# amikey/kaldi-ctc

Measured on AMD Instinct MI355X. Metric: CTC-train frames/sec, 5×BLSTM-512 mb=16, at 1/2/4/8 MI355X; loss match, higher is better.
Workload: dtype f32

## Files before the change

### include/ctc.h

```cpp
#ifndef KALDI_CTC_AMD_CTC_H_
#define KALDI_CTC_AMD_CTC_H_

#include <stddef.h>

#ifdef __cplusplus
extern "C" {
#endif

struct ihipStream_t;
typedef struct ihipStream_t *ctcStream_t;

typedef enum {
  CTC_STATUS_SUCCESS = 0,
  CTC_STATUS_MEMOPS_FAILED = 1,
  CTC_STATUS_INVALID_VALUE = 2,
  CTC_STATUS_EXECUTION_FAILED = 3,
  CTC_STATUS_UNKNOWN_ERROR = 4
} ctcStatus_t;

typedef enum { CTC_CPU = 0, CTC_GPU = 1 } ctcComputeLocation;

struct ctcOptions {
  ctcComputeLocation loc;
  union {
    unsigned int num_threads;
    ctcStream_t stream;
  };
  int blank_label;
};

int get_warpctc_version(void);
const char *ctcGetStatusString(ctcStatus_t status);

ctcStatus_t compute_ctc_loss(const float *const activations, float *gradients,
                             const int *const flat_labels, const int *const label_lengths,
                             const int *const input_lengths, int alphabet_size,
                             int minibatch, float *costs, void *workspace,
                             struct ctcOptions options);

ctcStatus_t get_workspace_size(const int *const label_lengths,
                               const int *const input_lengths, int alphabet_size,
                               int minibatch, struct ctcOptions info,
                               size_t *size_bytes);

ctcStatus_t mictc_compute_ctc_loss_async(const float *activations, float *gradients,
                                         const int *flat_labels, const int *label_lengths,
                                         const int *input_lengths, int alphabet_size,
                                         int minibatch, double *costs_dev, void *workspace,
                                         ctcStream_t stream, int blank_label);

int mictc_set_frame_group(int m);

int mictc_set_win(int on);

#ifdef __cplusplus
}
#endif
#endif
```

### kaldi-ctc_amd/__init__.py

```python
import ctypes
import os

import numpy as np

HERE = os.path.dirname(os.path.abspath(__file__))
LIB_PATH = os.path.join(HERE, "libkaldictc_amd.so")

CTC_CPU, CTC_GPU = 0, 1
CTC_STATUS = {0: "CTC_STATUS_SUCCESS", 1: "CTC_STATUS_MEMOPS_FAILED", 2: "CTC_STATUS_INVALID_VALUE",
              3: "CTC_STATUS_EXECUTION_FAILED", 4: "CTC_STATUS_UNKNOWN_ERROR"}

_lib = None


class CtcOptions(ctypes.Structure):
    _fields_ = [("loc", ctypes.c_int), ("stream", ctypes.c_void_p), ("blank_label", ctypes.c_int)]


class CtcError(RuntimeError):
    def __init__(self, status, where):
        msg = lib().ctcGetStatusString(status).decode()
        super().__init__(f"ctcStatus_t {status} : \"{msg}\" returned from '{where}'")
        self.status = status

# ... 86 lines not shown
    ll = np.ascontiguousarray(label_lengths, dtype=np.int32)
    il = np.ascontiguousarray(input_lengths, dtype=np.int32)
    opts = CtcOptions(CTC_GPU, None, 0)
    out = ctypes.c_size_t()
    st = lib().get_workspace_size(ll.ctypes.data, il.ctypes.data, int(alphabet_size), len(ll),
                                  opts, ctypes.byref(out))
    if st != 0:
        raise CtcError(st, "get_workspace_size")
    return out.value


def compute_ctc_loss(acts, flat_labels, label_lengths, input_lengths, want_grad=True, blank=0,
                     stream=None, workspace=None):
    import torch
    assert acts.is_cuda and acts.dtype == torch.float32 and acts.is_contiguous()
    T, N, A = acts.shape
    fl = np.ascontiguousarray(flat_labels, dtype=np.int32)
    if fl.size == 0:
        fl = np.zeros(1, np.int32)
    ll = np.ascontiguousarray(label_lengths, dtype=np.int32)
    il = np.ascontiguousarray(input_lengths, dtype=np.int32)
    if workspace is None:
        workspace = torch.empty(ctc_workspace_size(ll, il, A), dtype=torch.uint8, device=acts.device)
    grads = torch.empty_like(acts) if want_grad else None
    costs = np.zeros(N, np.float32)
    opts = CtcOptions(CTC_GPU, _stream_handle(stream), blank)
    st = lib().compute_ctc_loss(acts.data_ptr(), _ptr(grads), fl.ctypes.data, ll.ctypes.data,
                                il.ctypes.data, A, N, costs.ctypes.data, workspace.data_ptr(), opts)
    if st != 0:
        raise CtcError(st, "compute_ctc_loss")
    return costs, grads


class RnnError(RuntimeError):
    pass


def _krnn_check(st, where):
    if st != 0:
        raise RnnError(f"{where}: {lib().krnnGetStatusString(st).decode()} ({st})")


class Rnn:
    RELU, TANH, LSTM, GRU = 0, 1, 2, 3

    def __init__(self, mode, input_dim, hidden_dim, num_layers=1, bidirectional=True):
        self.mode, self.D, self.H, self.L = mode, input_dim, hidden_dim, num_layers
        self.dirs = 2 if bidirectional else 1
        h = ctypes.c_void_p()
        _krnn_check(lib().krnnCreate(ctypes.byref(h), mode, input_dim, hidden_dim, num_layers,
                                     1 if bidirectional else 0), "krnnCreate")
        self.h = h

    def set_precision(self, prec):
        _krnn_check(lib().krnnSetPrecision(self.h, 1 if prec in (1, "bf16") else 0), "krnnSetPrecision")

    def __del__(self):
        try:
            if self.h:
                lib().krnnDestroy(self.h)
        except Exception:
            pass

    @property
    def num_params(self):
        return lib().krnnGetParamsSize(self.h) // 4
# ... 904 lines not shown
```

### kaldi-ctc_amd/_bindings.py

```python
import ctypes

vp, ci, cl, cf, cd, sz = (ctypes.c_void_p, ctypes.c_int, ctypes.c_long, ctypes.c_float,
                          ctypes.c_double, ctypes.c_size_t)
ip = ctypes.POINTER(ctypes.c_int)

SIGS = {
    "krnnCreate": (ci, [ctypes.POINTER(vp), ci, ci, ci, ci, ci]),
    "krnnDestroy": (ci, [vp]),
    "krnnGetStatusString": (ctypes.c_char_p, [ci]),
    "krnnGetParamsSize": (sz, [vp]),
    "krnnGetLinLayerOffset": (cl, [vp, ci, ci, ci, ip]),
    "krnnGetWorkspaceSize": (sz, [vp, ci, ci]),
    "krnnGetTrainingReserveSize": (sz, [vp, ci, ci]),
    "krnnForwardTraining": (ci, [vp, vp, ci, ci, vp, vp, vp, vp, sz, vp, sz]),
    "krnnForwardInference": (ci, [vp, vp, ci, ci, vp, vp, vp, vp, sz]),
    "krnnGetInferenceSeqWorkspaceSize": (sz, [vp, ci, ci]),
    "krnnForwardInferenceSeq": (ci, [vp, vp, ci, ci, vp, vp, vp, vp, vp, sz]),
    "krnnBackwardData": (ci, [vp, vp, ci, ci, vp, vp, vp, vp, vp, sz, vp, sz]),
    "krnnBackwardWeights": (ci, [vp, vp, ci, ci, vp, vp, vp, sz, vp, vp, sz]),
    "krnnGetDeviceStatus": (ci, [vp, vp]),
    "kcm_add_mat_mat": (ci, [vp, ci, ci, ci, ci, ci, cf, vp, cl, vp, cl, cf, vp, cl]),
    "kcm_add_mat_mat_x3_workspace": (sz, [ci, ci, ci]),
    "kcm_add_mat_mat_x3": (ci, [vp, ci, ci, ci, ci, ci, cf, vp, cl, vp, cl, cf, vp, cl, vp]),
    "kcm_bench_gemm_packed": (cf, [vp, ci, ci, ci, ci, ci, ci]),
    "kcm_test_gemm_packed": (ci, [vp, ci, ci, ci, ci, ci, ci, ci, ci, vp, vp, vp, vp]),
    "kcm_test_row_stream": (ci, [vp, ci, ci, ci, ci, ci, vp, vp, vp, vp]),
    "kctc_test_component_side_streams": (ci, [vp, ci]),
    "kctc_test_rec6_select": (ci, [ci, ci, ci, ci, ci, ci, ip, ctypes.POINTER(vp)]),
    "kctc_test_rec_plan": (ci, [ci, ci, ci, ci, ci, ci, ctypes.POINTER(cl)]),
    "kcm_find_row_max_id": (ci, [vp, vp, cl, ci, vp]),
    "kcm_clip_gradient_rows": (ci, [vp, vp, cl, ci, cf, vp]),
    "kcm_add_vec_clipped": (ci, [vp, vp, vp, cl, cf, cf]),
    "kcm_add_row_sum_mat": (ci, [vp, vp, cl, ci, cf, cf, vp, vp]),
    "kctc_last_error": (ctypes.c_char_p, []),
    "kctc_nnet_create": (ci, [ctypes.POINTER(vp), ctypes.c_char_p, ctypes.c_ulonglong, ci]),
    "kctc_nnet_destroy": (ci, [vp]),
    "kctc_nnet_num_components": (ci, [vp]),
    "kctc_nnet_context": (ci, [vp, ip, ip]),
    "kctc_nnet_component_info": (ci, [vp, ci, ctypes.c_char_p, sz]),
    "kctc_nnet_num_params": (cl, [vp, ci]),
    "kctc_nnet_get_params": (ci, [vp, ci, vp, cl]),
    "kctc_nnet_set_params": (ci, [vp, ci, vp, cl]),
    "kctc_nnet_get_grad": (ci, [vp, ci, vp, cl]),
    "kctc_nnet_set_learning_rate": (ci, [vp, cf]),
    "kctc_nnet_clip_stats": (ci, [vp, ci, ctypes.POINTER(cd), ctypes.POINTER(cd)]),
    "kctc_nnet_srand": (ci, [vp, ctypes.c_uint]),
    "kctc_nnet_rand_calls": (ci, [vp, ctypes.POINTER(cl)]),
    "kctc_nnet_last_best_path": (ci, [vp, vp, cl]),
    "kctc_nnet_last_output": (ci, [vp, vp, cl]),
    "kctc_nnet_last_costs": (ci, [vp, vp, ci]),
    "kctc_nnet_train_step": (ci, [vp, vp, ci, ci, vp, vp, vp, ctypes.POINTER(cd), ctypes.POINTER(cd),
                                  ctypes.POINTER(cd)]),
    "kctc_nnet_compute_objf": (ci, [vp, vp, ci, ci, vp, vp, vp, ctypes.POINTER(cd), ctypes.POINTER(cd),
                                    ctypes.POINTER(cd)]),
    "kctc_nnet_train_step_async": (ci, [vp, vp, ci, ci, vp, vp, vp, ip, ctypes.POINTER(cd), ctypes.POINTER(cd),
                                        ctypes.POINTER(cd)]),
    "kctc_nnet_train_flush": (ci, [vp, ip, ctypes.POINTER(cd), ctypes.POINTER(cd), ctypes.POINTER(cd)]),
    "kctc_nnet_stream": (vp, [vp]),
    "kctc_nnet_set_profiling": (ci, [vp, ci]),
    "kctc_nnet_profile": (ci, [vp, ctypes.c_char_p, ctypes.POINTER(cd), ctypes.POINTER(ci)]),
    "kctc_nnet_write": (ci, [vp, ctypes.c_char_p]),
    "kctc_nnet_read": (ci, [ctypes.POINTER(vp), ctypes.c_char_p, ci]),
# ... 98 lines not shown
```

### kaldi-ctc_amd/csrc/common.h

```cpp
#pragma once
#include <hip/hip_runtime.h>

#include <cmath>
#include <cstdint>
#include <cstdio>
#include <stdexcept>
#include <string>

namespace kctc {

constexpr int kWave = 64;

struct HipError : std::runtime_error {
  explicit HipError(const std::string &s) : std::runtime_error(s) {}
};

#define KCTC_HIP_CHECK(expr)                                                          \
  do {                                                                                \
    hipError_t e_ = (expr);                                                           \
    if (e_ != hipSuccess)                                                             \
      throw ::kctc::HipError(std::string(#expr) + ": " + hipGetErrorString(e_) + " @" \
                             + __FILE__ + ":" + std::to_string(__LINE__));            \
  } while (0)

// ... 10 lines not shown
  for (int o = 32; o >= 1; o >>= 1) v = fmaxf(v, __shfl_xor(v, o, kWave));
  return v;
}
#define KCTC_DPP(v, ctrl, rm) \
  __int_as_float(__builtin_amdgcn_update_dpp(__float_as_int(v), __float_as_int(v), ctrl, rm, 0xF, false))
__device__ __forceinline__ float group_max8(float v) {
  v = fmaxf(v, KCTC_DPP(v, 0xB1, 0xF));
  v = fmaxf(v, KCTC_DPP(v, 0x4E, 0xF));
  v = fmaxf(v, KCTC_DPP(v, 0x141, 0xF));
  return v;
}
__device__ __forceinline__ float group_max16(float v) {
  v = group_max8(v);
  return fmaxf(v, KCTC_DPP(v, 0x140, 0xF));
}
__device__ __forceinline__ float wave_max_l63(float v) {
  v = group_max16(v);
  v = fmaxf(v, KCTC_DPP(v, 0x142, 0xA));
  v = fmaxf(v, KCTC_DPP(v, 0x143, 0xC));
  return v;
}

__device__ __forceinline__ float wave_sum(float v) {
#pragma unroll
  for (int o = 32; o >= 1; o >>= 1) v += __shfl_xor(v, o, kWave);
  return v;
}
__device__ __forceinline__ double wave_sum_d(double v) {
#pragma unroll
  for (int o = 32; o >= 1; o >>= 1) v += __shfl_xor(v, o, kWave);
  return v;
}

}
```

### kaldi-ctc_amd/csrc/ctc.hip

```cpp
#include <algorithm>
#include <cstring>
#include <type_traits>
#include <atomic>
#include <vector>

#include "common.h"
#include "ctc.h"
#include "prof.h"

namespace kctc {
namespace ctcimpl {

constexpr int kMaxLabel = 639;
constexpr int kThreads = 256;
constexpr int kABThreads = 512;
constexpr int kABWaves = kABThreads / 64;
constexpr int kSPT = (2 * kMaxLabel + 1 + kABThreads - 1) / kABThreads;
constexpr int kFR = 8;

struct UttDesc {
  int T, L, S, feasible, lab_off, pad;
  long long ab_off;
  long long off_off;
};

struct Layout {
  size_t desc, labels, links, owner, costs, logz, lp, spill, offs, total;
  int T_max;
  long long spill_floats, off_doubles;
};

static bool make_layout(const int *label_lengths, const int *input_lengths, int A, int N,
                        Layout *lay, std::vector<UttDesc> *descs, bool *bad) {
  *bad = false;
  if (A <= 0 || N <= 0 || !label_lengths || !input_lengths) { *bad = true; return false; }
  int T_max = 0;
  long long nlab = 0, spill = 0, offs = 0;
  if (descs) descs->resize(N);
  for (int n = 0; n < N; n++) {
    int T = input_lengths[n], L = label_lengths[n];
    if (T < 0 || L < 0 || L > kMaxLabel) { *bad = true; return false; }
    T_max = T > T_max ? T : T_max;
    int S = 2 * L + 1;
    if (descs) {
      UttDesc &d = (*descs)[n];
      d.T = T; d.L = L; d.S = S; d.feasible = 0; d.lab_off = (int)nlab; d.pad = 0;
      d.ab_off = spill; d.off_off = offs;
    }
    nlab += L;
    spill += 2LL * T * S;
    offs += 2LL * T;
  }
  Layout &l = *lay;
  size_t p = 0;
  l.desc = p;   p = align_up(p + sizeof(UttDesc) * N, 256);
  l.labels = p; p = align_up(p + sizeof(int) * (nlab > 0 ? nlab : 1), 256);
  l.links = p;  p = align_up(p + sizeof(int) * (nlab > 0 ? nlab : 1), 256);
  l.owner = p;  p = align_up(p + sizeof(int) * (size_t)N * A, 256);
  l.costs = p;  p = align_up(p + sizeof(double) * N, 256);
  l.logz = p;   p = align_up(p + sizeof(float) * (size_t)T_max * N + 4, 256);
  l.lp = p;     p = align_up(p + sizeof(float) * (size_t)T_max * N * A + 4, 256);
  l.spill = p;  p = align_up(p + sizeof(float) * (size_t)spill, 256);
  l.offs = p;   p = align_up(p + sizeof(double) * (size_t)offs, 256);
  l.total = p;
  l.T_max = T_max;
  l.spill_floats = spill;
  l.off_doubles = offs;
  return true;
}

__global__ __launch_bounds__(256) void ctc_logz(const float *__restrict__ acts, int A, long rows,
                                                float *__restrict__ logz, float *__restrict__ lp) {
  const long row = (long)blockIdx.x * 4 + (threadIdx.x >> 6);
  const int lane = threadIdx.x & 63;
  if (row >= rows) return;
  const float *r = acts + row * A;
  float m = -INFINITY;
  for (int a = lane; a < A; a += kWave) m = fmaxf(m, r[a]);
  m = wave_max(m);
  float s = 0.f;
  for (int a = lane; a < A; a += kWave) s += expf(r[a] - m);
  s = wave_sum(s);
  const float z = m + logf(s);
  if (lane == 0) logz[row] = z;
  for (int a = lane; a < A; a += kWave) lp[row * A + a] = r[a] - z;
}

__device__ __forceinline__ float fast_log1p(float x) {
  const float u = 1.f + x;
  return __builtin_fmaf(__builtin_amdgcn_logf(u), 0.693147180559945309f, x - (u - 1.f));
}
__device__ __forceinline__ float lse3(float a, float b, float c) {
  const float m = fmaxf(a, fmaxf(b, c));
  const float lo = fminf(a, fminf(b, c));
  const float md = fmaxf(fminf(a, b), fminf(fmaxf(a, b), c));
  const float r = m + fast_log1p(__expf(md - m) + __expf(lo - m));
  return m == -INFINITY ? -INFINITY : r;
}

struct AbLds {
  int F, SP, CP;
  int pair;
  __device__ __host__ size_t floats() const { return 2 * (size_t)F * SP + 2 * (size_t)CP + 2 * kABWaves + 4; }
};

__device__ __forceinline__ void lds_barrier() {
  asm volatile("s_waitcnt lgkmcnt(0)" ::: "memory");
  __builtin_amdgcn_s_barrier();
  asm volatile("" ::: "memory");
}

template <bool SPILL, int SPT, bool is_beta>
__device__ __forceinline__ void ab_body(
    const float *__restrict__ lp, int N, int A, int blank, UttDesc *__restrict__ descs,
    const int *__restrict__ labels, float *__restrict__ spill, double *__restrict__ offs,
    double *__restrict__ costs, AbLds lay) {
  const int n = is_beta ? blockIdx.x - N : blockIdx.x;
  const int tid = threadIdx.x, lane = tid & 63, wid = tid >> 6;
// ... 366 lines not shown
    lds_barrier();
  }
  if (!is_beta && tid == 0) {
    const float *pv = colb + (cur ^ 1) * CP;
    float a = pv[S - 1], b = S > 1 ? pv[S - 2] : -INFINITY;
    float m = fmaxf(a, b);
    double lpv = off + (double)m + log((double)expf(a - m) + (double)expf(b - m));
    costs[n] = -lpv;
  }
}

template <bool SPILL>
__global__ __launch_bounds__(64 * kWinWaves) void ctc_alpha_beta_win(
    const float *__restrict__ lp, int N, int A, int blank, UttDesc *__restrict__ descs,
    const int *__restrict__ labels, float *__restrict__ spill, double *__restrict__ offs,
    double *__restrict__ costs, AbLds lay) {
  if (blockIdx.x >= (unsigned)N) win_body<SPILL, true>(lp, N, A, blank, descs, labels, spill, offs, costs, lay);
  else win_body<SPILL, false>(lp, N, A, blank, descs, labels, spill, offs, costs, lay);
}

template <bool SPILL, int SPT>
__global__ __launch_bounds__(kABThreads) void ctc_alpha_beta(
    const float *__restrict__ lp, int N, int A, int blank, UttDesc *__restrict__ descs,
    const int *__restrict__ labels, float *__restrict__ spill, double *__restrict__ offs,
    double *__restrict__ costs, AbLds lay) {
  if (blockIdx.x >= (unsigned)N) ab_body<SPILL, SPT, true>(lp, N, A, blank, descs, labels, spill, offs, costs, lay);
  else ab_body<SPILL, SPT, false>(lp, N, A, blank, descs, labels, spill, offs, costs, lay);
}

__global__ __launch_bounds__(kThreads) void ctc_grad(
    const float *__restrict__ acts, const float *__restrict__ logz, float *__restrict__ grads,
    int N, int A, int T_max, int blank, const UttDesc *__restrict__ descs,
    const int *__restrict__ links, const int *__restrict__ owners, const float *__restrict__ spill,
    const double *__restrict__ offs, const double *__restrict__ costs) {
  extern __shared__ __attribute__((aligned(16))) char smem[];
  const int n = blockIdx.y, t0 = blockIdx.x * kFR, tid = threadIdx.x;
  const UttDesc d = descs[n];
  const int T = d.feasible ? d.T : 0, L = d.L, S = d.S;
  const int nf = min(kFR, T_max - t0);
  if (t0 >= T) {
    for (int it = tid; it < nf * A; it += kThreads) {
      int f = it / A, a = it - f * A;
      grads[((long)(t0 + f) * N + n) * A + a] = 0.f;
    }
    return;
  }
  float *occ = reinterpret_cast<float *>(smem);
  int *nxt = reinterpret_cast<int *>(occ + kFR * S);
  int *owner = nxt + (L > 0 ? L : 1);
  float *gblank = reinterpret_cast<float *>(owner + A);
  float *gtot = gblank + kFR;
  for (int a = tid; a < A; a += kThreads) owner[a] = owners[(long)n * A + a];
  for (int j = tid; j < L; j += kThreads) nxt[j] = links[d.lab_off + j];
  const double logp = -costs[n];
  const float *al = spill + d.ab_off;
  const float *be = al + (long long)T * S;
  const double *oa = offs + d.off_off, *ob = oa + T;
  const int nreal = min(nf, T - t0);
  for (int f = 0; f < nreal; f++) {
    const int t = t0 + f;
    const float Kt = (float)(oa[t] + ob[t] - logp);
    for (int s = tid; s < S; s += kThreads) {
      float v = al[(long)t * S + s] + be[(long)t * S + s];
      occ[f * S + s] = (v == -INFINITY) ? 0.f : expf(v + Kt);
    }
  }
  __syncthreads();
  {
    const int lane = tid & 63, wid = tid >> 6;
    for (int f = wid; f < nreal; f += kThreads / kWave) {
      float acc = 0.f, tot = 0.f;
      for (int s = 2 * lane; s < S; s += 2 * kWave) {
        acc += occ[f * S + s];
        tot += occ[f * S + s] + (s + 1 < S ? occ[f * S + s + 1] : 0.f);
      }
      acc = wave_sum(acc);
      tot = wave_sum(tot);
      if (lane == 0) { gblank[f] = acc / tot; gtot[f] = 1.f / tot; }
    }
  }
  __syncthreads();
  for (int it = tid; it < nf * A; it += kThreads) {
    const int f = it / A, a = it - f * A, t = t0 + f;
    const long idx = ((long)t * N + n) * A + a;
    float g = 0.f;
    if (t < T) {
      float gam = 0.f;
      if (a == blank) {
        gam = gblank[f];
      } else {
        for (int j = owner[a]; j >= 0; j = nxt[j]) gam += occ[f * S + 2 * j + 1];
        gam *= gtot[f];
      }
      g = expf(acts[idx] - logz[(long)t * N + n]) - gam;
    }
    grads[idx] = g;
  }
}

struct Staging {
  char *buf = nullptr;
  size_t cap = 0;
  hipEvent_t ev = nullptr;
  bool pending = false;
};
static thread_local Staging g_stage;

static char *staging_acquire(size_t bytes) {
  Staging &s = g_stage;
  if (s.pending) {
    if (hipEventSynchronize(s.ev) != hipSuccess) return nullptr;
    s.pending = false;
  }
  if (!s.ev && hipEventCreateWithFlags(&s.ev, hipEventDisableTiming) != hipSuccess) return nullptr;
  if (bytes > s.cap) {
    if (s.buf) (void)hipHostFree(s.buf);
    size_t cap = align_up(bytes * 2, 4096);
    if (hipHostMalloc((void **)&s.buf, cap, hipHostMallocDefault) != hipSuccess) {
      s.buf = nullptr; s.cap = 0;
      return nullptr;
    }
    s.cap = cap;
  }
  return s.buf;
}
static void staging_release(hipStream_t stream) {
  if (hipEventRecord(g_stage.ev, stream) == hipSuccess) g_stage.pending = true;
}

static std::atomic<int> g_frame_group{0};
static int frame_group() {
  int m = g_frame_group.load(std::memory_order_relaxed);
  if (m <= 0) {
    m = 8;
    int expect = 0;
    g_frame_group.compare_exchange_strong(expect, m);
    m = g_frame_group.load(std::memory_order_relaxed);
  }
  return m;
}

static std::atomic<int> g_win{1};
static bool win_enabled() { return g_win.load(std::memory_order_relaxed) != 0; }

static ctcStatus_t launch(const float *acts, float *grads, const int *flat_labels,
                          const int *label_lengths, const int *input_lengths, int A, int N,
                          double *costs_dev, void *workspace, hipStream_t stream, int blank) {
  Layout lay;
  std::vector<UttDesc> descs;
  bool bad = false;
  if (!make_layout(label_lengths, input_lengths, A, N, &lay, &descs, &bad) || bad)
    return CTC_STATUS_INVALID_VALUE;
  if (blank < 0 || blank >= A || !acts || !workspace) return CTC_STATUS_INVALID_VALUE;
  long long nlab = 0;
  for (int n = 0; n < N; n++) nlab += label_lengths[n];
  for (long long i = 0; i < nlab; i++)
    if (flat_labels[i] < 0 || flat_labels[i] >= A || flat_labels[i] == blank)
      return CTC_STATUS_INVALID_VALUE;
  char *ws = static_cast<char *>(workspace);
  char *stage = staging_acquire(lay.costs);
  if (!stage) return CTC_STATUS_MEMOPS_FAILED;
  memcpy(stage + lay.desc, descs.data(), sizeof(UttDesc) * N);
  if (nlab) memcpy(stage + lay.labels, flat_labels, sizeof(int) * nlab);
  {
    int *links = reinterpret_cast<int *>(stage + lay.links), *owner = reinterpret_cast<int *>(stage + lay.owner);
    std::fill(owner, owner + (size_t)N * A, -1);
    long long off = 0;
    for (int n = 0; n < N; n++) {
      const int L = label_lengths[n];
      int *own = owner + (size_t)n * A;
      for (int j = L - 1; j >= 0; j--) {
        const int k = flat_labels[off + j];
        links[off + j] = own[k];
        own[k] = j;
      }
      off += L;
    }
  }
  if (hipMemcpyAsync(ws, stage, lay.costs, hipMemcpyHostToDevice, stream) != hipSuccess)
    return CTC_STATUS_MEMOPS_FAILED;
  staging_release(stream);
  UttDesc *d_desc = reinterpret_cast<UttDesc *>(ws + lay.desc);
  const int *d_lab = reinterpret_cast<const int *>(ws + lay.labels);
  float *d_logz = reinterpret_cast<float *>(ws + lay.logz);
  float *d_spill = reinterpret_cast<float *>(ws + lay.spill);
  double *d_offs = reinterpret_cast<double *>(ws + lay.offs);
  const long rows = (long)lay.T_max * N;
  float *d_lp = reinterpret_cast<float *>(ws + lay.lp);
  if (rows > 0) {
    ProfSpan ps(stream, "ctc_logz");
    hipLaunchKernelGGL(ctc_logz, dim3(ceil_div(rows, 4)), dim3(256), 0, stream, acts, A, rows,
                       d_logz, d_lp);
  }
  const int want = grads != nullptr;
  {
    int Smax = 1;
    for (int n = 0; n < N; n++) Smax = 2 * label_lengths[n] + 1 > Smax ? 2 * label_lengths[n] + 1 : Smax;
    AbLds al;
    al.pair = frame_group();
    al.SP = (Smax + 63) / 64 * 64;
    const int own = 64 - 2 * (std::max(1, std::min(al.pair, 8)) - 1);
    const int nwv = std::max(1, (Smax + own - 1) / own);
    if (nwv <= kWinWaves && win_enabled()) {
      al.CP = std::max((Smax + 4 + 3) / 4 * 4, own * nwv);
      al.F = (int)std::min<size_t>(32, std::max<size_t>(4, (size_t)96 * 1024 / (2 * sizeof(float) * al.SP)));
      const size_t shm = sizeof(float) * (2 * (size_t)al.F * al.SP + 2 * (size_t)al.CP + 2 * kWinWaves + 4);
      if (shm > 160 * 1024) return CTC_STATUS_INVALID_VALUE;
      ProfSpan ps(stream, "ctc_alpha_beta");
      auto kern = want ? ctc_alpha_beta_win<true> : ctc_alpha_beta_win<false>;
      (void)hipFuncSetAttribute(reinterpret_cast<const void *>(kern), hipFuncAttributeMaxDynamicSharedMemorySize,
                                (int)shm);
      hipLaunchKernelGGL(kern, dim3(want ? 2 * N : N), dim3(64 * nwv), shm, stream, d_lp, N, A, blank, d_desc, d_lab,
                         d_spill, d_offs, costs_dev, al);
    } else {
      al.CP = std::max((Smax + 4 + 3) / 4 * 4, (Smax <= kABThreads ? 1 : kSPT) * kABThreads);
      al.F = (int)std::min<size_t>(32, std::max<size_t>(4, (size_t)96 * 1024 / (2 * sizeof(float) * al.SP)));
      const size_t shm = sizeof(float) * al.floats();
      if (shm > 160 * 1024) return CTC_STATUS_INVALID_VALUE;
      ProfSpan ps(stream, "ctc_alpha_beta");
      auto go = [&](auto kern, int grid) {
        (void)hipFuncSetAttribute(reinterpret_cast<const void *>(kern), hipFuncAttributeMaxDynamicSharedMemorySize,
                                  (int)shm);
        hipLaunchKernelGGL(kern, dim3(grid), dim3(kABThreads), shm, stream, d_lp, N, A, blank, d_desc, d_lab,
                           d_spill, d_offs, costs_dev, al);
      };
      if (Smax <= kABThreads) {
        if (want) go(ctc_alpha_beta<true, 1>, 2 * N);
        else go(ctc_alpha_beta<false, 1>, N);
      } else {
        if (want) go(ctc_alpha_beta<true, kSPT>, 2 * N);
        else go(ctc_alpha_beta<false, kSPT>, N);
      }
    }
  }
  if (want && lay.T_max > 0) {
    int Lmax = 0;
    for (int n = 0; n < N; n++) Lmax = label_lengths[n] > Lmax ? label_lengths[n] : Lmax;
    const int Smax = 2 * Lmax + 1;
    size_t shm = sizeof(float) * kFR * Smax + sizeof(int) * (Lmax > 0 ? Lmax : 1) +
                 sizeof(int) * A + 2 * sizeof(float) * kFR;
    if (shm > 160 * 1024) return CTC_STATUS_INVALID_VALUE;
    ProfSpan ps(stream, "ctc_grad");
    hipLaunchKernelGGL(ctc_grad, dim3(ceil_div(lay.T_max, kFR), N), dim3(kThreads), shm, stream,
                       acts, d_logz, grads, N, A, lay.T_max, blank, d_desc,
                       reinterpret_cast<const int *>(ws + lay.links), reinterpret_cast<const int *>(ws + lay.owner),
                       d_spill, d_offs, costs_dev);
  }
  if (hipGetLastError() != hipSuccess) return CTC_STATUS_EXECUTION_FAILED;
  return CTC_STATUS_SUCCESS;
}

}
}

using namespace kctc::ctcimpl;

extern "C" {

int get_warpctc_version(void) { return 2; }

int mictc_set_frame_group(int m) {
  const int prev = frame_group();
  if (m > 0) g_frame_group.store(std::max(1, std::min(m, 8)));
  return prev;
}

int mictc_set_win(int on) {
  const int prev = g_win.load();
  if (on >= 0) g_win.store(on ? 1 : 0);
  return prev;
}

const char *ctcGetStatusString(ctcStatus_t status) {
  switch (status) {
    case CTC_STATUS_SUCCESS: return "no error";
    case CTC_STATUS_MEMOPS_FAILED: return "cuda memcpy or memset failed";
    case CTC_STATUS_INVALID_VALUE: return "invalid value";
    case CTC_STATUS_EXECUTION_FAILED: return "execution failed";
    case CTC_STATUS_UNKNOWN_ERROR:
    default: return "unknown error";
  }
}

ctcStatus_t get_workspace_size(const int *const label_lengths, const int *const input_lengths,
                               int alphabet_size, int minibatch, struct ctcOptions info,
                               size_t *size_bytes) {
  if (!size_bytes || info.loc != CTC_GPU) return CTC_STATUS_INVALID_VALUE;
  Layout lay;
  bool bad = false;
  if (!make_layout(label_lengths, input_lengths, alphabet_size, minibatch, &lay, nullptr, &bad) ||
      bad)
    return CTC_STATUS_INVALID_VALUE;
  *size_bytes = lay.total;
  return CTC_STATUS_SUCCESS;
}

ctcStatus_t mictc_compute_ctc_loss_async(const float *activations, float *gradients,
                                         const int *flat_labels, const int *label_lengths,
                                         const int *input_lengths, int alphabet_size,
                                         int minibatch, double *costs_dev, void *workspace,
                                         ctcStream_t stream, int blank_label) {
  if (!costs_dev) return CTC_STATUS_INVALID_VALUE;
  try {
    return launch(activations, gradients, flat_labels, label_lengths, input_lengths,
                  alphabet_size, minibatch, costs_dev, workspace,
                  reinterpret_cast<hipStream_t>(stream), blank_label);
  } catch (...) {
    return CTC_STATUS_UNKNOWN_ERROR;
  }
}

ctcStatus_t compute_ctc_loss(const float *const activations, float *gradients,
                             const int *const flat_labels, const int *const label_lengths,
                             const int *const input_lengths, int alphabet_size, int minibatch,
                             float *costs, void *workspace, struct ctcOptions options) {
  if (options.loc != CTC_GPU || !costs) return CTC_STATUS_INVALID_VALUE;
  Layout lay;
  bool bad = false;
  if (!make_layout(label_lengths, input_lengths, alphabet_size, minibatch, &lay, nullptr, &bad) ||
      bad)
    return CTC_STATUS_INVALID_VALUE;
  hipStream_t stream = reinterpret_cast<hipStream_t>(options.stream);
  double *d_costs = reinterpret_cast<double *>(static_cast<char *>(workspace) + lay.costs);
  ctcStatus_t st = mictc_compute_ctc_loss_async(activations, gradients, flat_labels,
                                                label_lengths, input_lengths, alphabet_size,
                                                minibatch, d_costs, workspace, options.stream,
                                                options.blank_label);
  if (st != CTC_STATUS_SUCCESS) return st;
  std::vector<double> hc(minibatch);
  if (hipMemcpyAsync(hc.data(), d_costs, sizeof(double) * minibatch, hipMemcpyDeviceToHost,
                     stream) != hipSuccess)
    return CTC_STATUS_MEMOPS_FAILED;
  if (hipStreamSynchronize(stream) != hipSuccess) return CTC_STATUS_EXECUTION_FAILED;
  for (int n = 0; n < minibatch; n++) costs[n] = (float)hc[n];
  return CTC_STATUS_SUCCESS;
}

}
```

### kaldi-ctc_amd/csrc/elementwise.hip

```cpp
#include "common.h"
#include "elementwise.h"

namespace kctc {
namespace {

typedef float floatx4 __attribute__((ext_vector_type(4)));

__global__ __launch_bounds__(256) void k_clip_sgd(float *__restrict__ w, const float *__restrict__ dw,
                                                  long n, float lr, float clip, const unsigned *skip) {
  if (skip && *skip) return;
  const long n4 = n / 4;
  const long stride = (long)gridDim.x * 256;
  const bool vec = ((uintptr_t)w % 16 == 0) && ((uintptr_t)dw % 16 == 0);
  long i = (long)blockIdx.x * 256 + threadIdx.x;
  if (vec) {
    for (; i < n4; i += stride) {
      floatx4 g = reinterpret_cast<const floatx4 *>(dw)[i];
      floatx4 v = reinterpret_cast<floatx4 *>(w)[i];
#pragma unroll
      for (int j = 0; j < 4; j++) {
        float x = g[j];
        if (clip > 0.f) x = fminf(fmaxf(x, -clip), clip);
        v[j] += lr * x;
      }
// ... 24 lines not shown
        ss += v[0] * v[0] + v[1] * v[1] + v[2] * v[2] + v[3] * v[3];
      }
    } else {
      for (int j = lane; j < dim; j += 64) ss += r[j] * r[j];
    }
    ss = wave_sum(ss);
    const float sc = ss * inv_thr2;
    if (!(sc < 1.f)) {
      clipped = 1;
      const float f = rsqrtf(sc);
      if (vec) {
        for (int j = lane; j < dim / 4; j += 64) {
          floatx4 v = reinterpret_cast<const floatx4 *>(r)[j];
          reinterpret_cast<floatx4 *>(r)[j] = v * f;
        }
      } else {
        for (int j = lane; j < dim; j += 64) r[j] *= f;
      }
    }
  }
  if (lane == 0) cnt[threadIdx.x >> 6] = clipped;
  __syncthreads();
  if (threadIdx.x == 0) {
    int c = cnt[0] + cnt[1] + cnt[2] + cnt[3];
    if (c) atomicAdd(nclipped, c);
  }
}

__global__ __launch_bounds__(256) void k_row_argmax(const float *__restrict__ m, long rows, int cols,
                                                    int *__restrict__ ids) {
  const long row = (long)blockIdx.x * 4 + (threadIdx.x >> 6);
  const int lane = threadIdx.x & 63;
  if (row >= rows) return;
  const float *r = m + row * cols;
  float v[4];
  int vi[4];
#pragma unroll
  for (int k = 0; k < 4; k++) {
    v[k] = -1e20f;
    vi[k] = -1;
    for (int j = lane + 64 * k; j < cols; j += 256) {
      const float x = r[j];
      if (x > v[k]) { v[k] = x; vi[k] = j; }
    }
  }
  if (v[2] > v[0]) { v[0] = v[2]; vi[0] = vi[2]; }
  if (v[3] > v[1]) { v[1] = v[3]; vi[1] = vi[3]; }
  if (v[1] > v[0]) { v[0] = v[1]; vi[0] = vi[1]; }
  float b = v[0];
  int bi = vi[0];
#pragma unroll
  for (int w = 32; w >= 1; w >>= 1) {
    const float ob = __shfl_down(b, w, 64);
    const int oi = __shfl_down(bi, w, 64);
    if (ob > b) { b = ob; bi = oi; }
  }
  if (lane == 0) ids[row] = bi;
}

__global__ __launch_bounds__(256) void k_sum_rows(const float *__restrict__ X, long rows, int cols,
                                                  float alpha, float beta, float *__restrict__ out) {
  __shared__ float part[16][64];
  const int c = blockIdx.x * 64 + (threadIdx.x & 63), g = threadIdx.x >> 6;
  float s = 0.f;
  if (c < cols)
    for (long r = blockIdx.y * 4 + g; r < rows; r += 4L * gridDim.y) s += X[r * cols + c];
  part[g][threadIdx.x & 63] = s;
  __syncthreads();
  if (g == 0 && c < cols) {
    float v = ((part[0][threadIdx.x] + part[1][threadIdx.x]) + part[2][threadIdx.x]) + part[3][threadIdx.x];
    out[(long)blockIdx.y * cols + c] = v;
  }
}

__global__ __launch_bounds__(256) void k_sum_partials(const float *__restrict__ part, int nparts,
                                                      int cols, float alpha, float beta,
                                                      float *__restrict__ out) {
  const int c = blockIdx.x * 256 + threadIdx.x;
  if (c >= cols) return;
  float s = 0.f;
  for (int p = 0; p < nparts; p++) s += part[(long)p * cols + c];
  out[c] = alpha * s + (beta != 0.f ? beta * out[c] : 0.f);
}

__global__ void k_scale(float *p, long n, float a) {
  for (long i = (long)blockIdx.x * 256 + threadIdx.x; i < n; i += (long)gridDim.x * 256) p[i] *= a;
}

__global__ void k_fill(float *p, long n, float v) {
// ... 247 lines not shown
```

### kaldi-ctc_amd/csrc/nnet.cpp

```cpp
#include "nnet.h"
#include "kaldi_io.h"

#include <algorithm>
#include <cmath>
#include <cstdio>
#include <cstring>
#include <iomanip>
#include <iostream>
#include <sstream>

#include "common.h"
#include "ctc.h"
#include "decodable.h"
#include "dropout.h"
#include "elementwise.h"
#include "gemm.h"
#include "prof.h"

namespace kctc {
namespace nnet2 {

int levenshtein(const int *ref, int m, const int *hyp, int n) {
  if (m <= 0) return n > 0 ? n : 0;
  if (n <= 0) return m;
// ... 1502 lines not shown
      r->ClearPackedInput();
      r->PropagateSeq(in, &out, num_frames);
    } else {
      comp.Propagate(chunk_info_[c], chunk_info_[c + 1], in, &out);
    }
  }
  unsigned herr = 0;
  KCTC_HIP_CHECK(hipMemcpyAsync(&herr, err_word_.p, sizeof(unsigned), hipMemcpyDeviceToHost, S()));
  KCTC_HIP_CHECK(hipStreamSynchronize(S()));
  if (herr) throw std::runtime_error("recurrence hand-off timed out (device error word set)");
  return forward_data_[C];
}

void NnetCtcUpdater::Enqueue(const float *feats, int T_max, int N, const int *num_frames,
                             const int *flat_labels, const int *label_lengths) {
  if (pending_ == 2) throw std::logic_error("two minibatches already queued");
  const int C = nnet_->NumComponents();
  if (N <= 0 || T_max <= 0) throw std::invalid_argument("empty minibatch");
  const long rows = (long)T_max * N;
  set_minibatch(nnet_, N);
  err_word_.ensure(256);
  KCTC_HIP_CHECK(hipMemsetAsync(err_word_.p, 0, sizeof(unsigned), S()));
  if (inject_err_) {
    KCTC_HIP_CHECK(hipMemcpyAsync(err_word_.p, &inject_err_, sizeof(unsigned), hipMemcpyHostToDevice, S()));
    KCTC_HIP_CHECK(hipStreamSynchronize(S()));
    inject_err_ = 0;
  }
  for (int c = 0; c < C; c++)
    if (auto *r = dynamic_cast<CuDNNRecurrentComponent *>(&nnet_->GetComponent(c)))
      r->SetErrorWord(static_cast<unsigned *>(err_word_.p));
  forward_data_.resize(C + 1);
  SetupChunks(T_max, N);
  forward_data_[0].SetView(const_cast<float *>(feats), rows * nnet_->NumSplice(), nnet_->InputDim());
  Propagate(T_max, N);

  const CuMatrixBase &out = forward_data_[C];
  const int A = nnet_->OutputDim();
  for (int n = 0; n < N; n++)
    if (label_lengths[n] < 0) throw std::invalid_argument("negative label length");
  size_t ws = 0;
  {
    ctcOptions o;
    o.loc = CTC_GPU;
    o.stream = reinterpret_cast<ctcStream_t>(S());
    o.blank_label = 0;
    ctcStatus_t st = get_workspace_size(label_lengths, num_frames, A, N, o, &ws);
    if (st != CTC_STATUS_SUCCESS)
      throw std::runtime_error(std::string("get_workspace_size: ") + ctcGetStatusString(st));
    if (ws > ctc_ws_.bytes) {
      std::vector<int> worst_l(N, std::min(T_max, 639)), worst_t(N, T_max);
      size_t w2 = 0;
      if (get_workspace_size(worst_l.data(), worst_t.data(), A, N, o, &w2) == CTC_STATUS_SUCCESS)
        ws = std::max(ws, w2);
    }
  }
  ctc_ws_.ensure(ws);
  costs_dev_.ensure(sizeof(double) * N);
  ids_dev_.ensure(sizeof(int) * rows);
  CuMatrix &deriv = deriv_a_;
  deriv.Resize(rows, A);
  {
    ProfScope ps("layer_ctc");
    ctcStatus_t st = mictc_compute_ctc_loss_async(out.Data(), update_ ? deriv.Data() : nullptr,
                                                  flat_labels, label_lengths, num_frames, A, N,
                                                  static_cast<double *>(costs_dev_.p), ctc_ws_.p,
                                                  reinterpret_cast<ctcStream_t>(S()), 0);
    if (st != CTC_STATUS_SUCCESS)
      throw std::runtime_error(std::string("compute_ctc_loss: ") + ctcGetStatusString(st));
  }
  {
    ProfScope ps("argmax");
    row_argmax(S(), out.Data(), rows, A, static_cast<int *>(ids_dev_.p));
  }
  if (update_) Backprop(T_max, N);

  Slot &sl = slots_[next_];
  const size_t need = sizeof(double) * N + sizeof(int) * rows + sizeof(unsigned) * C;
  if (need > sl.bytes) {
    if (sl.pinned) {
      if (sl.ev) KCTC_HIP_CHECK(hipEventSynchronize(sl.ev));
      (void)hipHostFree(sl.pinned);
    }
    KCTC_HIP_CHECK(hipHostMalloc((void **)&sl.pinned, need, hipHostMallocDefault));
    sl.bytes = need;
  }
  if (!sl.ev) KCTC_HIP_CHECK(hipEventCreateWithFlags(&sl.ev, hipEventDisableTiming));
  double *hcost = reinterpret_cast<double *>(sl.pinned);
  int *hids = reinterpret_cast<int *>(sl.pinned + sizeof(double) * N);
  unsigned *herr = reinterpret_cast<unsigned *>(hids + rows);
  KCTC_HIP_CHECK(hipMemcpyAsync(hcost, costs_dev_.p, sizeof(double) * N, hipMemcpyDeviceToHost, S()));
  KCTC_HIP_CHECK(hipMemcpyAsync(hids, ids_dev_.p, sizeof(int) * rows, hipMemcpyDeviceToHost, S()));
  sl.nerr = 1;
  KCTC_HIP_CHECK(hipMemcpyAsync(herr, err_word_.p, sizeof(unsigned), hipMemcpyDeviceToHost, S()));
  KCTC_HIP_CHECK(hipEventRecord(sl.ev, S()));
  sl.N = N;
  sl.rows = rows;
  sl.num_frames.assign(num_frames, num_frames + N);
  long nlab = 0;
  for (int n = 0; n < N; n++) nlab += label_lengths[n];
  sl.labels.assign(flat_labels, flat_labels + nlab);
  sl.label_lengths.assign(label_lengths, label_lengths + N);
  next_ ^= 1;
  pending_++;
}

// ... 76 lines not shown
      const void *rows = nullptr, *cols = nullptr;
      if (below && below->Desc().prec == r->Desc().prec) below->PackedOutput(&rows, &cols);
      r->SetPackedInput(rows, cols);
      if (!below) r->ClearInputBound();
      r->SetPrepackDx(update_ && c > first);
      r->SetPrepackW(update_ && c >= first);
      below = r;
    } else if (!comp.IsIdentityForward()) {
      below = nullptr;
    }
    const CuMatrixBase &in = forward_data_[c];
    CuMatrix &out = forward_data_[c + 1];
    if (comp.IsIdentityForward()) {
      out.SetView(in.Data(), in.NumRows(), comp.OutputDim());
      continue;
    }
    out.Resize((long)T * N, comp.OutputDim());
    const auto *rnn = dynamic_cast<const CuDNNRecurrentComponent *>(&comp);
    const CuDNNRecurrentComponent *next = nullptr;
    if (rnn) {
      int c2 = c + 1;
      while (c2 < C && nnet_->GetComponent(c2).IsIdentityForward()) c2++;
      if (c2 < C) next = dynamic_cast<const CuDNNRecurrentComponent *>(&nnet_->GetComponent(c2));
    }
    if (next) rnn->PropagateChained(in, &out, *next);
    else comp.Propagate(chunk_info_[c], chunk_info_[c + 1], in, &out);
  }
}

void NnetCtcUpdater::Backprop(int T, int N) {
  const int C = nnet_->NumComponents();
  const long rows = (long)T * N;
  const int A = nnet_->OutputDim();
  {
    ProfScope ps("scale");
    scale_inplace(S(), deriv_a_.Data(), rows * (long)A, -1.f);
  }
  CuMatrix *cur = &deriv_a_, *other = &deriv_b_;
  const int first = nnet_->FirstUpdatableComponent();
  int max_dim = A;
  for (int c = 0; c <= C; c++) max_dim = std::max(max_dim, chunk_info_[c].feat_dim);
  std::vector<int> updated;
  for (int c = C - 1; c >= first; c--) {
    Component &comp = nnet_->GetComponent(c);
    const CuMatrixBase &in = forward_data_[c], &outv = forward_data_[c + 1];
    Component *to_update = &comp;
    const bool need_in_deriv = c > first;
    CuMatrixBase *in_deriv = nullptr;
    CuMatrixBase view;
    if (need_in_deriv) {
      if (comp.IsIdentityForward()) {
        view = CuMatrixBase(cur->Data(), rows, comp.InputDim());
        in_deriv = &view;
      } else {
        other->Resize(rows, std::max(comp.InputDim(), max_dim));
        view = CuMatrixBase(other->Data(), rows, comp.InputDim());
        in_deriv = &view;
      }
    }
    if (auto *cg = dynamic_cast<ClipGradientComponent *>(&comp)) {
      cg->rng_ = &repair_rng_;
      if (cg->Shadow()) to_update = cg->Shadow();
    }
    const CuMatrixBase od(cur->Data(), rows, comp.OutputDim());
    const bool rec = exchange_ && dynamic_cast<CuDNNRecurrentComponent *>(&comp);
    if (rec) exchange_->BeforeRecurrence(S());
    comp.Backprop(chunk_info_[c], chunk_info_[c + 1], in, outv, od, to_update, in_deriv);
    if (rec) exchange_->AfterRecurrence();
    if (comp.IsUpdatable()) {
      auto *u = static_cast<UpdatableComponent *>(&comp);
// ... 23 lines not shown
```

Before: 858,600.

## Fuse argmax into CTC logz, negate gradients in-kernel, hoist CTC prep before forward

The row argmax is computed inside the ctc_logz kernel, which already reads every activation row. Gradient negation moves into ctc_grad through a flag, so the separate scale_inplace pass over the derivative matrix goes away. CTC preparation (label upload, layout setup) is split out and issued before the forward propagation, so its host work and H2D copy sit ahead of the network compute. The aim is to cut extra full passes over the output matrix and kernel launches; the cost is a slightly heavier logz kernel, plus a fallback argmax launch for any rows beyond the longest utterance.

New measurement: 861,400 (median of 3 runs). Within noise of the previous version (+0.3%).

```diff
diff --git a/include/ctc.h b/include/ctc.h
--- a/include/ctc.h
+++ b/include/ctc.h
@@ -49,6 +49,15 @@
                                          int minibatch, double *costs_dev, void *workspace,
                                          ctcStream_t stream, int blank_label);
 
+#define MICTC_NEGATE_GRADIENTS 1
+ctcStatus_t mictc_ctc_prepare(const int *flat_labels, const int *label_lengths,
+                              const int *input_lengths, int alphabet_size, int minibatch,
+                              void *workspace, ctcStream_t stream, int blank_label);
+ctcStatus_t mictc_ctc_run(const float *activations, float *gradients, const int *label_lengths,
+                          const int *input_lengths, int alphabet_size, int minibatch,
+                          double *costs_dev, void *workspace, ctcStream_t stream, int blank_label,
+                          int flags, int *row_ids_dev);
+
 int mictc_set_frame_group(int m);
 
 int mictc_set_win(int on);
diff --git a/kaldi-ctc_amd/__init__.py b/kaldi-ctc_amd/__init__.py
--- a/kaldi-ctc_amd/__init__.py
+++ b/kaldi-ctc_amd/__init__.py
@@ -142,6 +142,56 @@
     return costs, grads
 
 
+MICTC_NEGATE_GRADIENTS = 1
+
+
+def _ctc_host_args(flat_labels, label_lengths, input_lengths):
+    fl = np.ascontiguousarray(flat_labels, dtype=np.int32)
+    if fl.size == 0:
+        fl = np.zeros(1, np.int32)
+    return (fl, np.ascontiguousarray(label_lengths, dtype=np.int32),
+            np.ascontiguousarray(input_lengths, dtype=np.int32))
+
+
+def ctc_prepare(flat_labels, label_lengths, input_lengths, alphabet_size, workspace, blank=0, stream=None):
+    fl, ll, il = _ctc_host_args(flat_labels, label_lengths, input_lengths)
+    st = lib().mictc_ctc_prepare(fl.ctypes.data, ll.ctypes.data, il.ctypes.data, int(alphabet_size), len(ll),
+                                 workspace.data_ptr(), _stream_handle(stream), blank)
+    if st != 0:
+        raise CtcError(st, "mictc_ctc_prepare")
+
+
+def ctc_run(acts, label_lengths, input_lengths, workspace, costs_dev, want_grad=True, blank=0, negate=False,
+            want_ids=False, stream=None):
+    import torch
+    assert acts.is_cuda and acts.dtype == torch.float32 and acts.is_contiguous()
+    T, N, A = acts.shape
+    ll = np.ascontiguousarray(label_lengths, dtype=np.int32)
+    il = np.ascontiguousarray(input_lengths, dtype=np.int32)
+    grads = torch.empty_like(acts) if want_grad else None
+    ids = torch.empty(T * N, dtype=torch.int32, device=acts.device) if want_ids else None
+    st = lib().mictc_ctc_run(acts.data_ptr(), _ptr(grads), ll.ctypes.data, il.ctypes.data, A, N,
+                             costs_dev.data_ptr(), workspace.data_ptr(), _stream_handle(stream), blank,
+                             MICTC_NEGATE_GRADIENTS if negate else 0, _ptr(ids))
+    if st != 0:
+        raise CtcError(st, "mictc_ctc_run")
+    return grads, ids
+
+
+def ctc_logz(acts2d, want_ids=False, stream=None):
+    import torch
+    assert acts2d.is_cuda and acts2d.dtype == torch.float32 and acts2d.is_contiguous()
+    rows, A = acts2d.shape
+    logz = torch.empty(rows, dtype=torch.float32, device=acts2d.device)
+    lp = torch.empty_like(acts2d)
+    ids = torch.empty(rows, dtype=torch.int32, device=acts2d.device) if want_ids else None
+    st = lib().kctc_test_ctc_logz(_stream_handle(stream), acts2d.data_ptr(), A, rows, logz.data_ptr(),
+                                  lp.data_ptr(), _ptr(ids))
+    if st != 0:
+        raise KctcError(f"kctc_test_ctc_logz failed ({st})")
+    return logz, lp, ids
+
+
 class RnnError(RuntimeError):
     pass
 
diff --git a/kaldi-ctc_amd/_bindings.py b/kaldi-ctc_amd/_bindings.py
--- a/kaldi-ctc_amd/_bindings.py
+++ b/kaldi-ctc_amd/_bindings.py
@@ -28,6 +28,9 @@
     "kctc_test_component_side_streams": (ci, [vp, ci]),
     "kctc_test_rec6_select": (ci, [ci, ci, ci, ci, ci, ci, ip, ctypes.POINTER(vp)]),
     "kctc_test_rec_plan": (ci, [ci, ci, ci, ci, ci, ci, ctypes.POINTER(cl)]),
+    "kctc_test_ctc_logz": (ci, [vp, vp, ci, cl, vp, vp, vp]),
+    "mictc_ctc_prepare": (ci, [vp, vp, vp, ci, ci, vp, vp, ci]),
+    "mictc_ctc_run": (ci, [vp, vp, vp, vp, ci, ci, vp, vp, vp, ci, ci, vp]),
     "kcm_find_row_max_id": (ci, [vp, vp, cl, ci, vp]),
     "kcm_clip_gradient_rows": (ci, [vp, vp, cl, ci, cf, vp]),
     "kcm_add_vec_clipped": (ci, [vp, vp, vp, cl, cf, cf]),
diff --git a/kaldi-ctc_amd/csrc/common.h b/kaldi-ctc_amd/csrc/common.h
--- a/kaldi-ctc_amd/csrc/common.h
+++ b/kaldi-ctc_amd/csrc/common.h
@@ -66,4 +66,30 @@
   return v;
 }
 
+__device__ __forceinline__ int row_argmax_wave(const float *__restrict__ r, int cols, int lane) {
+  float v[4];
+  int vi[4];
+#pragma unroll
+  for (int k = 0; k < 4; k++) {
+    v[k] = -1e20f;
+    vi[k] = -1;
+    for (int j = lane + 64 * k; j < cols; j += 256) {
+      const float x = r[j];
+      if (x > v[k]) { v[k] = x; vi[k] = j; }
+    }
+  }
+  if (v[2] > v[0]) { v[0] = v[2]; vi[0] = vi[2]; }
+  if (v[3] > v[1]) { v[1] = v[3]; vi[1] = vi[3]; }
+  if (v[1] > v[0]) { v[0] = v[1]; vi[0] = vi[1]; }
+  float b = v[0];
+  int bi = vi[0];
+#pragma unroll
+  for (int w = 32; w >= 1; w >>= 1) {
+    const float ob = __shfl_down(b, w, 64);
+    const int oi = __shfl_down(bi, w, 64);
+    if (ob > b) { b = ob; bi = oi; }
+  }
+  return bi;
 }
+
+}
diff --git a/kaldi-ctc_amd/csrc/ctc.hip b/kaldi-ctc_amd/csrc/ctc.hip
--- a/kaldi-ctc_amd/csrc/ctc.hip
+++ b/kaldi-ctc_amd/csrc/ctc.hip
@@ -7,6 +7,7 @@
 #include "common.h"
 #include "ctc.h"
 #include "prof.h"
+#include "test_hooks.h"
 
 namespace kctc {
 namespace ctcimpl {
@@ -70,7 +71,8 @@
 }
 
 __global__ __launch_bounds__(256) void ctc_logz(const float *__restrict__ acts, int A, long rows,
-                                                float *__restrict__ logz, float *__restrict__ lp) {
+                                                float *__restrict__ logz, float *__restrict__ lp,
+                                                int *__restrict__ ids) {
   const long row = (long)blockIdx.x * 4 + (threadIdx.x >> 6);
   const int lane = threadIdx.x & 63;
   if (row >= rows) return;
@@ -84,6 +86,10 @@
   const float z = m + logf(s);
   if (lane == 0) logz[row] = z;
   for (int a = lane; a < A; a += kWave) lp[row * A + a] = r[a] - z;
+  if (ids) {
+    const int bi = row_argmax_wave(r, A, lane);
+    if (lane == 0) ids[row] = bi;
+  }
 }
 
 __device__ __forceinline__ float fast_log1p(float x) {
@@ -516,16 +522,17 @@
     const float *__restrict__ acts, const float *__restrict__ logz, float *__restrict__ grads,
     int N, int A, int T_max, int blank, const UttDesc *__restrict__ descs,
     const int *__restrict__ links, const int *__restrict__ owners, const float *__restrict__ spill,
-    const double *__restrict__ offs, const double *__restrict__ costs) {
+    const double *__restrict__ offs, const double *__restrict__ costs, int negate) {
   extern __shared__ __attribute__((aligned(16))) char smem[];
   const int n = blockIdx.y, t0 = blockIdx.x * kFR, tid = threadIdx.x;
+  const float zero = negate ? -0.f : 0.f;
   const UttDesc d = descs[n];
   const int T = d.feasible ? d.T : 0, L = d.L, S = d.S;
   const int nf = min(kFR, T_max - t0);
   if (t0 >= T) {
     for (int it = tid; it < nf * A; it += kThreads) {
       int f = it / A, a = it - f * A;
-      grads[((long)(t0 + f) * N + n) * A + a] = 0.f;
+      grads[((long)(t0 + f) * N + n) * A + a] = zero;
     }
     return;
   }
@@ -578,7 +585,7 @@
       }
       g = expf(acts[idx] - logz[(long)t * N + n]) - gam;
     }
-    grads[idx] = g;
+    grads[idx] = negate ? -g : g;
   }
 }
 
@@ -627,15 +634,14 @@
 static std::atomic<int> g_win{1};
 static bool win_enabled() { return g_win.load(std::memory_order_relaxed) != 0; }
 
-static ctcStatus_t launch(const float *acts, float *grads, const int *flat_labels,
-                          const int *label_lengths, const int *input_lengths, int A, int N,
-                          double *costs_dev, void *workspace, hipStream_t stream, int blank) {
+static ctcStatus_t prepare(const int *flat_labels, const int *label_lengths, const int *input_lengths,
+                           int A, int N, void *workspace, hipStream_t stream, int blank) {
   Layout lay;
   std::vector<UttDesc> descs;
   bool bad = false;
   if (!make_layout(label_lengths, input_lengths, A, N, &lay, &descs, &bad) || bad)
     return CTC_STATUS_INVALID_VALUE;
-  if (blank < 0 || blank >= A || !acts || !workspace) return CTC_STATUS_INVALID_VALUE;
+  if (blank < 0 || blank >= A || !workspace) return CTC_STATUS_INVALID_VALUE;
   long long nlab = 0;
   for (int n = 0; n < N; n++) nlab += label_lengths[n];
   for (long long i = 0; i < nlab; i++)
@@ -664,6 +670,18 @@
   if (hipMemcpyAsync(ws, stage, lay.costs, hipMemcpyHostToDevice, stream) != hipSuccess)
     return CTC_STATUS_MEMOPS_FAILED;
   staging_release(stream);
+  return CTC_STATUS_SUCCESS;
+}
+
+static ctcStatus_t run(const float *acts, float *grads, const int *label_lengths,
+                       const int *input_lengths, int A, int N, double *costs_dev, void *workspace,
+                       hipStream_t stream, int blank, int flags, int *row_ids) {
+  Layout lay;
+  bool bad = false;
+  if (!make_layout(label_lengths, input_lengths, A, N, &lay, nullptr, &bad) || bad)
+    return CTC_STATUS_INVALID_VALUE;
+  if (blank < 0 || blank >= A || !acts || !workspace) return CTC_STATUS_INVALID_VALUE;
+  char *ws = static_cast<char *>(workspace);
   UttDesc *d_desc = reinterpret_cast<UttDesc *>(ws + lay.desc);
   const int *d_lab = reinterpret_cast<const int *>(ws + lay.labels);
   float *d_logz = reinterpret_cast<float *>(ws + lay.logz);
@@ -674,7 +692,7 @@
   if (rows > 0) {
     ProfSpan ps(stream, "ctc_logz");
     hipLaunchKernelGGL(ctc_logz, dim3(ceil_div(rows, 4)), dim3(256), 0, stream, acts, A, rows,
-                       d_logz, d_lp);
+                       d_logz, d_lp, row_ids);
   }
   const int want = grads != nullptr;
   {
@@ -728,7 +746,7 @@
     hipLaunchKernelGGL(ctc_grad, dim3(ceil_div(lay.T_max, kFR), N), dim3(kThreads), shm, stream,
                        acts, d_logz, grads, N, A, lay.T_max, blank, d_desc,
                        reinterpret_cast<const int *>(ws + lay.links), reinterpret_cast<const int *>(ws + lay.owner),
-                       d_spill, d_offs, costs_dev);
+                       d_spill, d_offs, costs_dev, (flags & MICTC_NEGATE_GRADIENTS) ? 1 : 0);
   }
   if (hipGetLastError() != hipSuccess) return CTC_STATUS_EXECUTION_FAILED;
   return CTC_STATUS_SUCCESS;
@@ -764,6 +782,13 @@
     case CTC_STATUS_UNKNOWN_ERROR:
     default: return "unknown error";
   }
+}
+
+int kctc_test_ctc_logz(struct ihipStream_t *stream, const float *acts, int A, long rows, float *logz, float *lp,
+                       int *ids) {
+  if (!acts || !logz || !lp || A <= 0 || rows <= 0) return 1;
+  hipLaunchKernelGGL(ctc_logz, dim3(kctc::ceil_div(rows, 4)), dim3(256), 0, stream, acts, A, rows, logz, lp, ids);
+  return hipGetLastError() == hipSuccess ? 0 : 3;
 }
 
 ctcStatus_t get_workspace_size(const int *const label_lengths, const int *const input_lengths,
@@ -785,10 +810,33 @@
                                          int minibatch, double *costs_dev, void *workspace,
                                          ctcStream_t stream, int blank_label) {
   if (!costs_dev) return CTC_STATUS_INVALID_VALUE;
+  ctcStatus_t st = mictc_ctc_prepare(flat_labels, label_lengths, input_lengths, alphabet_size,
+                                     minibatch, workspace, stream, blank_label);
+  if (st != CTC_STATUS_SUCCESS) return st;
+  return mictc_ctc_run(activations, gradients, label_lengths, input_lengths, alphabet_size,
+                       minibatch, costs_dev, workspace, stream, blank_label, 0, nullptr);
+}
+
+ctcStatus_t mictc_ctc_prepare(const int *flat_labels, const int *label_lengths,
+                              const int *input_lengths, int alphabet_size, int minibatch,
+                              void *workspace, ctcStream_t stream, int blank_label) {
   try {
-    return launch(activations, gradients, flat_labels, label_lengths, input_lengths,
-                  alphabet_size, minibatch, costs_dev, workspace,
-                  reinterpret_cast<hipStream_t>(stream), blank_label);
+    return prepare(flat_labels, label_lengths, input_lengths, alphabet_size, minibatch, workspace,
+                   reinterpret_cast<hipStream_t>(stream), blank_label);
+  } catch (...) {
+    return CTC_STATUS_UNKNOWN_ERROR;
+  }
+}
+
+ctcStatus_t mictc_ctc_run(const float *activations, float *gradients, const int *label_lengths,
+                          const int *input_lengths, int alphabet_size, int minibatch,
+                          double *costs_dev, void *workspace, ctcStream_t stream, int blank_label,
+                          int flags, int *row_ids_dev) {
+  if (!costs_dev) return CTC_STATUS_INVALID_VALUE;
+  try {
+    return run(activations, gradients, label_lengths, input_lengths, alphabet_size, minibatch,
+               costs_dev, workspace, reinterpret_cast<hipStream_t>(stream), blank_label, flags,
+               row_ids_dev);
   } catch (...) {
     return CTC_STATUS_UNKNOWN_ERROR;
   }
diff --git a/kaldi-ctc_amd/csrc/elementwise.hip b/kaldi-ctc_amd/csrc/elementwise.hip
--- a/kaldi-ctc_amd/csrc/elementwise.hip
+++ b/kaldi-ctc_amd/csrc/elementwise.hip
@@ -80,29 +80,7 @@
   const long row = (long)blockIdx.x * 4 + (threadIdx.x >> 6);
   const int lane = threadIdx.x & 63;
   if (row >= rows) return;
-  const float *r = m + row * cols;
-  float v[4];
-  int vi[4];
-#pragma unroll
-  for (int k = 0; k < 4; k++) {
-    v[k] = -1e20f;
-    vi[k] = -1;
-    for (int j = lane + 64 * k; j < cols; j += 256) {
-      const float x = r[j];
-      if (x > v[k]) { v[k] = x; vi[k] = j; }
-    }
-  }
-  if (v[2] > v[0]) { v[0] = v[2]; vi[0] = vi[2]; }
-  if (v[3] > v[1]) { v[1] = v[3]; vi[1] = vi[3]; }
-  if (v[1] > v[0]) { v[0] = v[1]; vi[0] = vi[1]; }
-  float b = v[0];
-  int bi = vi[0];
-#pragma unroll
-  for (int w = 32; w >= 1; w >>= 1) {
-    const float ob = __shfl_down(b, w, 64);
-    const int oi = __shfl_down(bi, w, 64);
-    if (ob > b) { b = ob; bi = oi; }
-  }
+  const int bi = row_argmax_wave(m + row * cols, cols, lane);
   if (lane == 0) ids[row] = bi;
 }
 
diff --git a/kaldi-ctc_amd/csrc/nnet.cpp b/kaldi-ctc_amd/csrc/nnet.cpp
--- a/kaldi-ctc_amd/csrc/nnet.cpp
+++ b/kaldi-ctc_amd/csrc/nnet.cpp
@@ -1558,9 +1558,6 @@
   forward_data_.resize(C + 1);
   SetupChunks(T_max, N);
   forward_data_[0].SetView(const_cast<float *>(feats), rows * nnet_->NumSplice(), nnet_->InputDim());
-  Propagate(T_max, N);
-
-  const CuMatrixBase &out = forward_data_[C];
   const int A = nnet_->OutputDim();
   for (int n = 0; n < N; n++)
     if (label_lengths[n] < 0) throw std::invalid_argument("negative label length");
@@ -1581,22 +1578,29 @@
     }
   }
   ctc_ws_.ensure(ws);
+  {
+    ctcStatus_t st = mictc_ctc_prepare(flat_labels, label_lengths, num_frames, A, N, ctc_ws_.p,
+                                       reinterpret_cast<ctcStream_t>(S()), 0);
+    if (st != CTC_STATUS_SUCCESS)
+      throw std::runtime_error(std::string("compute_ctc_loss: ") + ctcGetStatusString(st));
+  }
+  Propagate(T_max, N);
+  const CuMatrixBase &out = forward_data_[C];
   costs_dev_.ensure(sizeof(double) * N);
   ids_dev_.ensure(sizeof(int) * rows);
   CuMatrix &deriv = deriv_a_;
   deriv.Resize(rows, A);
   {
     ProfScope ps("layer_ctc");
-    ctcStatus_t st = mictc_compute_ctc_loss_async(out.Data(), update_ ? deriv.Data() : nullptr,
-                                                  flat_labels, label_lengths, num_frames, A, N,
-                                                  static_cast<double *>(costs_dev_.p), ctc_ws_.p,
-                                                  reinterpret_cast<ctcStream_t>(S()), 0);
+    ctcStatus_t st = mictc_ctc_run(out.Data(), update_ ? deriv.Data() : nullptr, label_lengths,
+                                   num_frames, A, N, static_cast<double *>(costs_dev_.p), ctc_ws_.p,
+                                   reinterpret_cast<ctcStream_t>(S()), 0, MICTC_NEGATE_GRADIENTS,
+                                   static_cast<int *>(ids_dev_.p));
     if (st != CTC_STATUS_SUCCESS)
       throw std::runtime_error(std::string("compute_ctc_loss: ") + ctcGetStatusString(st));
-  }
-  {
-    ProfScope ps("argmax");
-    row_argmax(S(), out.Data(), rows, A, static_cast<int *>(ids_dev_.p));
+    const long seen = (long)*std::max_element(num_frames, num_frames + N) * N;
+    if (seen < rows)
+      row_argmax(S(), out.Data() + seen * A, rows - seen, A, static_cast<int *>(ids_dev_.p) + seen);
   }
   if (update_) Backprop(T_max, N);
 
@@ -1739,10 +1743,6 @@
   const int C = nnet_->NumComponents();
   const long rows = (long)T * N;
   const int A = nnet_->OutputDim();
-  {
-    ProfScope ps("scale");
-    scale_inplace(S(), deriv_a_.Data(), rows * (long)A, -1.f);
-  }
   CuMatrix *cur = &deriv_a_, *other = &deriv_b_;
   const int first = nnet_->FirstUpdatableComponent();
   int max_dim = A;
```
